# gillesdegottex/percivaltts

Hardware: AMD Instinct MI355X
Metric: acoustic frames/sec per WGAN-GP critic+gen step (higher is better)
Workload: dtype f32

## Files before the change

### include/percival_hip.h

```cpp
#ifndef PERCIVAL_HIP_H
#define PERCIVAL_HIP_H

#include <stddef.h>
#include <stdint.h>

#ifdef __cplusplus
extern "C" {
#endif

#define PTTS_OK            0
#define PTTS_EINVAL       -1
#define PTTS_ELAUNCH      -2
#define PTTS_EWORKSPACE   -3
#define PTTS_EDEVICE      -4

#define PTTS_IN_NONE     0
#define PTTS_IN_LRELU    1
#define PTTS_IN_MASKMUL  2

#define PTTS_PAD_SAME    0
#define PTTS_PAD_CAUSAL  1

#define PTTS_ACT_NONE    0
#define PTTS_ACT_LRELU   1
// ... 136 lines not shown
int ptts_dense_bf16x6_res(const float* A, const void* planes, const float* bias, float* C, int M, int N, int K,
                          long long lda, long long ldc, int in_mode, const float* in_scale, const float* in_shift,
                          const float* mask_src, float alpha, const float* res, int res_rows, long long ldr,
                          const float* out_mask, void* stream);
int ptts_dense_bf16x6_stats_rows(int M, int N);
int ptts_dense_bf16x6_stats(const float* A, const void* planes, const float* bias, float* C, int M, int N, int K,
                            long long lda, long long ldc, int in_mode, const float* in_scale, const float* in_shift,
                            float alpha, double* stats, int capacity_rows, int* nrows_out, void* stream);
int ptts_dense_bf16x6_bwd_affine(const float* A, const void* planes, float* C, int M, int N, int K, long long lda, long long ldc,
                                 const float* z, const float* scale, const float* shift, float alpha,
                                 double* stats, int capacity_rows, int* nrows_out, void* stream);
int ptts_partial_rows_sum(const double* partials, int nrows, int ncols, double* out, void* stream);
int ptts_dft_mirror(float* Ap, int NB, int B, int Cin, int Kh, void* stream);

int ptts_conv1d_freq_kernel_planes(const float* w, const float* tw, void* planes, int NB, int KW, int Cin, int N, int Kh, void* stream);

int ptts_transpose_batched(const float* src, float* dst, int nb, int rows, int cols, void* stream);
int ptts_conv1d_freq_wgrad_combine(const float* out2, float* dW, int KW, int Cin, int N, int Kh, void* stream);

size_t ptts_conv1d_freq_wgrad_inverse_workspace_bytes(int KW, int Cin, int N);
int ptts_conv1d_freq_wgrad_inverse(const float* Gt, const float* t2, float* dW, void* workspace, size_t workspace_bytes,
                                   int NB, int NBp, int KW, int Cin, int N, int Kh, void* stream);

int ptts_dense_bf16x6_batched(const float* A, long long strideA, const void* planes, long long stride_planes_bytes,
                              const float* bias, float* C, long long strideC, int nbatch, int M, int N, int K,
                              long long lda, long long ldc, int planes_count, void* stream);

int ptts_split3_frames(const float* x, void* p1, void* p2, void* p3, int B, int T, int C, int pad_left, int pad_right,
                       int Cp, void* stream);
int ptts_split3_weight_t(const float* w, void* p1, void* p2, void* p3, int KW, int C, int N, int Cp, void* stream);
int ptts_conv1d_bf16x6(const void* a1, const void* a2, const void* a3, const void* bt1, const void* bt2, const void* bt3,
                       const float* bias, float* y, int B, int T, int KW, int Cp, int N, void* stream);

int ptts_split3_frames_t(const float* x, void* p1, void* p2, void* p3, int B, int T, int C, int pad_left, int Tp, int Crows,
                         long long Pp, void* stream);
int ptts_conv1d_wgrad_bf16x6(const void* xt1, const void* xt2, const void* xt3, const void* yt1, const void* yt2,
                             const void* yt3, float* dw, int B, int T, int KW, int C, int N, int Crows, long long Pp,
                             void* stream);

int ptts_transpose_frames(const float* x, float* out, int B, int T, int C, int pad_left, int Tp, int Crows, long long Pp,
                          void* stream);
int ptts_conv1d_wgrad_t(const float* xt, const float* yt, float* dw, float* db, int B, int T, int KW, int C, int N, int Crows,
                        long long Pp, void* stream);

size_t ptts_colstats_workspace_bytes(long long rows, int C);
int ptts_colstats(const float* x, long long rows, int C,
// ... 144 lines not shown
```

### percivaltts_amd/_hip.py

```python
import ctypes
import os
import re

import torch

_HERE = os.path.dirname(os.path.abspath(__file__))
LIB_PATH = os.environ.get('PTTS_LIB_PATH') or os.path.join(_HERE, 'lib', 'libpercival_hip.so')
HEADER_PATH = os.environ.get('PTTS_HEADER_PATH') or os.path.join(_HERE, '..', 'include', 'percival_hip.h')


class HipLibraryError(RuntimeError):
    pass


_SCALARS = {'int': ctypes.c_int, 'unsigned': ctypes.c_uint, 'float': ctypes.c_float, 'double': ctypes.c_double,
            'size_t': ctypes.c_size_t, 'long long': ctypes.c_longlong, 'unsigned long long': ctypes.c_ulonglong}
_DECLARATOR = re.compile(r'(.*[\s*])(\w+)\s*(\[\s*\])?', re.S)


def _ctype(spelling, where):
    t = ' '.join(w for w in spelling.replace('*', ' * ').split() if w != 'const')
    if t.endswith('*'):
        return ctypes.c_char_p if t == 'char *' else ctypes.c_void_p
    if t not in _SCALARS:
# ... 32 lines not shown
        args = [] if m.group(3).strip() == 'void' else [_declaration(a, decl)[1] for a in m.group(3).split(',')]
        functions[m.group(2)] = (_ctype(m.group(1), decl), args)
    return structs, functions


def read_header(path):
    if not os.path.exists(path):
        raise HipLibraryError('percival_hip.h not found at {}: it lies in include/ beside the package (or set PTTS_HEADER_PATH). '
                              'The binding is read from it.'.format(path))
    with open(path) as f:
        return parse_header(f.read())


_STRUCTS, SIGNATURES = read_header(HEADER_PATH)


def _structure(name, cname):
    return type(name, (ctypes.Structure,), {'_fields_': _STRUCTS[cname], '__doc__': 'struct {} of include/percival_hip.h.'.format(cname)})


WGradDesc = _structure('WGradDesc', 'ptts_wgrad_desc')
DenseWgradReduceDesc = _structure('DenseWgradReduceDesc', 'ptts_dense_wgrad_reduce_desc')
DenseSplitDesc = _structure('DenseSplitDesc', 'ptts_dense_split_desc')
Conv2dReduceDesc = _structure('Conv2dReduceDesc', 'ptts_conv2d_reduce_desc')

_lib = None


def lib():
    global _lib
    if _lib is None:
        if not os.path.exists(LIB_PATH):
            raise HipLibraryError(
                'libpercival_hip.so not found at {}: run `python -c "import __graft_entry__ as g; g.build()"` '
                '(or `make -C percivaltts_amd/csrc`). There is no CPU fallback.'.format(LIB_PATH))
        l = ctypes.CDLL(LIB_PATH)
        for name, (res, args) in SIGNATURES.items():
            fn = getattr(l, name)
            fn.restype = res
            fn.argtypes = args
        if os.environ.get('PTTS_DETERMINISTIC', '0') == '1':
            l.ptts_set_deterministic(1)
        _lib = l
    return _lib


# ... 83 lines not shown
```

### percivaltts_amd/csrc/dense.hip

```cpp
#include "common.h"
#include <cstdlib>

namespace ptts {
namespace dns {

typedef __bf16 bf16x8 __attribute__((ext_vector_type(8)));
typedef __bf16 bf16x4 __attribute__((ext_vector_type(4)));
typedef __bf16 bf16x2 __attribute__((ext_vector_type(2)));
typedef float f32x4 __attribute__((ext_vector_type(4)));
typedef float f32x2 __attribute__((ext_vector_type(2)));
typedef unsigned u32x2 __attribute__((ext_vector_type(2)));
typedef unsigned short u16;

constexpr int THREADS = 512;
constexpr int NBLK = 256;
constexpr int BK = 32;

#define DNS_PRODUCTS(X) X(2, 0) X(1, 1) X(0, 2) X(1, 0) X(0, 1) X(0, 0)
#define DNS_PRODUCTS_NPL(NPL, X) do { if (NPL == 3) { X(2, 0) X(1, 1) X(0, 2) X(1, 0) X(0, 1) } X(0, 0) } while (0)

__device__ __forceinline__ unsigned pk_bf16(float a, float b) {
    return __builtin_bit_cast(unsigned, __builtin_convertvector((f32x2){a, b}, bf16x2));
}
__device__ __forceinline__ void split3_pair(float a, float b, unsigned& p1, unsigned& p2, unsigned& p3) {
    p1 = pk_bf16(a, b);
    const float ra = a - __builtin_bit_cast(float, p1 << 16), rb = b - __builtin_bit_cast(float, p1 & 0xffff0000u);
    p2 = pk_bf16(ra, rb);
    const float sa = ra - __builtin_bit_cast(float, p2 << 16), sb = rb - __builtin_bit_cast(float, p2 & 0xffff0000u);
    p3 = pk_bf16(sa, sb);
}
__device__ __forceinline__ float max_fast(float a, float b) {
    float r;
    asm("v_max_f32 %0, %1, %2" : "=v"(r) : "v"(a), "v"(b));
    return r;
// ... 171 lines not shown
#pragma unroll
        for (int h = 0; h < 4; ++h) split3_pair(v[2 * h], v[2 * h + 1], q[0][h], q[1][h], q[2][h]);
        const size_t idx = ((size_t)nt * a.KS + ks) * 64 + lane;
#pragma unroll
        for (int p = 0; p < 3; ++p)
            *reinterpret_cast<uint4*>(planes + p * ps + idx * 8) = make_uint4(q[p][0], q[p][1], q[p][2], q[p][3]);
    }
}

#ifndef DNS_DEPTH
#define DNS_DEPTH 2
#endif
struct DenseArgs {
    const float* A; const float* mask_src; const float* in_scale; const float* in_shift;
    const u16* planes; const float* bias; const float* out_mask; float* C;
    int M, N, K, NT, KS;
    long long lda, ldc;
    float alpha, out_alpha;
    int accumulate, has_affine, vec_out;
    const float* res; int res_rows; long long ldr;
    long long bsA, bsP, bsC;
    double* stats;
    const float* om_scale; const float* om_shift;
};

template <int MODE, bool AFFINE, int MT, int NPL>
__global__ __launch_bounds__(THREADS) void dense_bf16x6_kernel(DenseArgs g) {
    if (gridDim.z > 1) {
        g.A += (long long)blockIdx.z * g.bsA;
        g.planes += (long long)blockIdx.z * g.bsP;
        g.C += (long long)blockIdx.z * g.bsC;
    }
    constexpr int TBM = 16 * MT;
    constexpr int NA = (TBM * 8 + THREADS - 1) / THREADS;
    constexpr int ROWS = NA * THREADS / 8;
    constexpr int PL = ROWS * BK;
    constexpr bool MASK = MODE == PTTS_IN_MASKMUL;
    __shared__ __attribute__((aligned(16))) u16 As[2][NPL * PL];
    const int tid = threadIdx.x, lane = tid & 63;
    const int wave = __builtin_amdgcn_readfirstlane(tid >> 6);
    const int li = lane & 15, lg = lane >> 4;
    const int m0 = blockIdx.x * TBM, n0 = blockIdx.y * NBLK;
    const int KS = g.KS;
    const bool wave_live = n0 + 32 * wave < g.N;

    const int kq = tid & 7;
    const float* pa[NA]; const float* pm[NA]; bool oka[NA]; int dst[NA];
#pragma unroll
    for (int j = 0; j < NA; ++j) {
        const int row = (tid + j * THREADS) >> 3;
        oka[j] = row < TBM && m0 + row < g.M;
        const long long base = (long long)(oka[j] ? m0 + row : 0) * g.lda + 4 * kq;
        pa[j] = g.A + base;
        pm[j] = MASK ? g.mask_src + base : nullptr;
        dst[j] = row * BK + ((((kq >> 1) ^ ((row >> 1) & 2))) << 3) + (kq & 1) * 4;
// ... 35 lines not shown
                unsigned a1, a2, a3, b1, b2, b3;
                split3_pair(a[0], a[1], a1, a2, a3);
                split3_pair(a[2], a[3], b1, b2, b3);
                *reinterpret_cast<u32x2*>(d) = (u32x2){a1, b1};
                *reinterpret_cast<u32x2*>(d + PL) = (u32x2){a2, b2};
                *reinterpret_cast<u32x2*>(d + 2 * PL) = (u32x2){a3, b3};
            } else {
                *reinterpret_cast<u32x2*>(d) = (u32x2){pk_bf16(a[0], a[1]), pk_bf16(a[2], a[3])};
            }
        }
    };

    const size_t ps = (size_t)g.NT * KS * 512;
    const u16* wp[2];
#pragma unroll
    for (int j = 0; j < 2; ++j) wp[j] = g.planes + (((size_t)((n0 >> 4) + 2 * (wave_live ? wave : 0) + j) * KS) * 64 + lane) * 8;
    auto load_w = [&](int s, bf16x8 (&wf)[2][NPL]) {
#pragma unroll
        for (int j = 0; j < 2; ++j)
#pragma unroll
            for (int p = 0; p < NPL; ++p) wf[j][p] = *reinterpret_cast<const bf16x8*>(wp[j] + p * ps + (size_t)s * 512);
    };

    f32x4 acc[MT][2];
#pragma unroll
    for (int i = 0; i < MT; ++i) { acc[i][0] = f32x4{0.f, 0.f, 0.f, 0.f}; acc[i][1] = f32x4{0.f, 0.f, 0.f, 0.f}; }
    const int boff = li * BK + ((lg ^ ((li >> 1) & 2)) << 3);
    auto mfma_rows = [&](const u16* as, const bf16x8 (&wf)[2][NPL], int i0, int i1) {
#pragma unroll
        for (int i = i0; i < i1; ++i) {
            bf16x8 bf[NPL];
#pragma unroll
            for (int p = 0; p < NPL; ++p) bf[p] = *reinterpret_cast<const bf16x8*>(as + p * PL + boff + i * 16 * BK);
#define DNS_MM(PA, PW)                                                                                    \
            acc[i][0] = __builtin_amdgcn_mfma_f32_16x16x32_bf16(wf[0][PW < NPL ? PW : 0], bf[PA < NPL ? PA : 0], acc[i][0], 0, 0, 0);    \
            acc[i][1] = __builtin_amdgcn_mfma_f32_16x16x32_bf16(wf[1][PW < NPL ? PW : 0], bf[PA < NPL ? PA : 0], acc[i][1], 0, 0, 0);
            DNS_PRODUCTS_NPL(NPL, DNS_MM);
#undef DNS_MM
        }
    };

    constexpr int DEPTH = DNS_DEPTH;
    Stage sg[DEPTH];
    bf16x8 wc[2][NPL], wn[2][NPL];
#pragma unroll
    for (int j = 0; j < DEPTH; ++j) load_a(j, sg[j]);
    load_w(0, wc);
    commit(sg[0], As[0]);
    load_a(DEPTH, sg[0]);
    __syncthreads();
    auto step = [&](int s, int cut, Stage& nx) {
        const u16* as = As[s & 1];
        load_w(s + 1 < KS ? s + 1 : s, wn);
        mfma_rows(as, wc, 0, cut);
        commit(nx, As[(s + 1) & 1]);
        load_a(s + 1 + DEPTH, nx);
        mfma_rows(as, wc, cut, MT);
#pragma unroll
        for (int j = 0; j < 2; ++j)
#pragma unroll
            for (int p = 0; p < NPL; ++p) wc[j][p] = wn[j][p];
        __syncthreads();
    };
    auto run = [&](int cut) {
        int s = 0;
        for (; s + DEPTH <= KS; s += DEPTH) {
#pragma unroll
            for (int j = 0; j < DEPTH; ++j) step(s + j, cut, sg[(j + 1) % DEPTH]);
        }
#pragma unroll
        for (int j = 0; j < DEPTH; ++j)
            if (s + j < KS) step(s + j, cut, sg[(j + 1) % DEPTH]);
    };
    if (wave < 4) run(2); else run(MT - 2);
    if (!wave_live) return;
    const bool interior = m0 + TBM <= g.M;
    if (!g.vec_out) {
#pragma unroll
        for (int j = 0; j < 2; ++j)
#pragma unroll
            for (int i = 0; i < MT; ++i) {
                const int m = m0 + 16 * i + li;
                if (m >= g.M) continue;
#pragma unroll
                for (int e = 0; e < 4; ++e) {
                    const int n = n0 + 32 * wave + 16 * j + 4 * lg + e;
                    if (n >= g.N) continue;
                    const long long off = (long long)m * g.ldc + n;
                    float v = acc[i][j][e] + (g.bias ? g.bias[n] : 0.f);
                    if (g.out_mask) v *= g.out_mask[off] > 0.f ? 1.f : g.out_alpha;
                    if (g.res) { int mr = m; while (mr >= g.res_rows) mr -= g.res_rows; v += g.res[(long long)mr * g.ldr + n]; }
                    g.C[off] = v;
                }
            }
        return;
    }
#pragma unroll
    for (int j = 0; j < 2; ++j) {
        const int n = n0 + 32 * wave + 16 * j + 4 * lg;
        if (n >= g.N) continue;
        f32x4 bv = {0.f, 0.f, 0.f, 0.f};
        if (g.bias) bv = *reinterpret_cast<const f32x4*>(g.bias + n);
        const long long off0 = (long long)(m0 + li) * g.ldc + n;
        auto res_at = [&](int m) { int mr = m; while (mr >= g.res_rows) mr -= g.res_rows; return g.res + (long long)mr * g.ldr + n; };
        f32x4 ssum = {0.f, 0.f, 0.f, 0.f}, ssq = {0.f, 0.f, 0.f, 0.f};
        f32x4 osc = {1.f, 1.f, 1.f, 1.f}, osh = {0.f, 0.f, 0.f, 0.f};
        if (g.om_scale) { osc = *reinterpret_cast<const f32x4*>(g.om_scale + n); osh = *reinterpret_cast<const f32x4*>(g.om_shift + n); }
        auto aff_store = [&](f32x4& v, const f32x4& z) {
#pragma unroll
            for (int e = 0; e < 4; ++e) {
                const float gd = v[e] * ((z[e] * osc[e] + osh[e]) > 0.f ? 1.f : g.out_alpha);
                ssum[e] += gd * z[e]; ssq[e] += gd;
                v[e] = gd * osc[e];
            }
        };
        if (interior) {
            f32x4 mk[MT], old[MT];
            if (g.out_mask) {
#pragma unroll
                for (int i = 0; i < MT; ++i) mk[i] = *reinterpret_cast<const f32x4*>(g.out_mask + off0 + (long long)16 * i * g.ldc);
            }
            if (g.res) {
#pragma unroll
                for (int i = 0; i < MT; ++i) old[i] = *reinterpret_cast<const f32x4*>(res_at(m0 + 16 * i + li));
            }
#pragma unroll
            for (int i = 0; i < MT; ++i) {
                f32x4 v = acc[i][j] + bv;
                if (g.om_scale) {
                    aff_store(v, mk[i]);
                } else if (g.out_mask) {
#pragma unroll
                    for (int e = 0; e < 4; ++e) v[e] = v[e] * (mk[i][e] > 0.f ? 1.f : g.out_alpha);
                }
                if (g.res) v += old[i];
                if (g.stats && !g.om_scale) { ssum += v; ssq += v * v; }
                *reinterpret_cast<f32x4*>(g.C + off0 + (long long)16 * i * g.ldc) = v;
            }
        } else {
#pragma unroll
            for (int i = 0; i < MT; ++i) {
                const int m = m0 + 16 * i + li;
                if (m >= g.M) continue;
                const long long off = off0 + (long long)16 * i * g.ldc;
                f32x4 v = acc[i][j] + bv;
                if (g.out_mask) {
                    const f32x4 mk = *reinterpret_cast<const f32x4*>(g.out_mask + off);
                    if (g.om_scale) {
                        aff_store(v, mk);
                    } else {
#pragma unroll
                        for (int e = 0; e < 4; ++e) v[e] = v[e] * (mk[e] > 0.f ? 1.f : g.out_alpha);
                    }
                }
                if (g.res) v += *reinterpret_cast<const f32x4*>(res_at(m));
                if (g.stats && !g.om_scale) { ssum += v; ssq += v * v; }
                *reinterpret_cast<f32x4*>(g.C + off) = v;
            }
        }
        if (g.stats) {
#pragma unroll
            for (int e = 0; e < 4; ++e)
#pragma unroll
                for (int m = 1; m < 16; m <<= 1) { ssum[e] += __shfl_xor(ssum[e], m, 64); ssq[e] += __shfl_xor(ssq[e], m, 64); }
            if (li == 0) {
                double* row = g.stats + (size_t)blockIdx.x * 2 * g.N;
#pragma unroll
                for (int e = 0; e < 4; ++e) { row[n + e] = (double)ssum[e]; row[g.N + n + e] = (double)ssq[e]; }
            }
        }
    }
}

static int pick_mt(int M, int col_blocks) {
    static int forced = -1;
    if (forced < 0) { const char* e = getenv("PTTS_DENSE_MT"); forced = e ? atoi(e) : 0; }
    if (forced >= 4 && forced <= 8) return forced;
    int best = 8; double best_eff = -1.0;
    for (int mt = 4; mt <= 8; ++mt) {
        const long long blocks = (long long)((M + 16 * mt - 1) / (16 * mt)) * col_blocks;
// ... 370 lines not shown
                        const float* out_mask, double* stats, int stats_capacity_rows, int* stats_rows_out, void* stream) {
    const int accumulate = res != nullptr;
    PTTS_REQUIRE(!res || (res_rows > 0 && ldr >= N && M <= 8LL * res_rows), "dense_bf16x6: bad residual (rows %d, ldr %lld)", res_rows, ldr);
    PTTS_REQUIRE(A && planes && C, "dense_bf16x6: null matrix");
    PTTS_REQUIRE(ptts_dense_bf16x6_supported(M, N, K, lda, ldc), "dense_bf16x6: unsupported shape M=%d N=%d K=%d lda=%lld ldc=%lld (K and lda must be multiples of 4)", M, N, K, lda, ldc);
    PTTS_REQUIRE(lda >= K && ldc >= N, "dense_bf16x6: bad leading dims");
    PTTS_REQUIRE(in_mode >= 0 && in_mode <= 2, "dense_bf16x6: bad in_mode %d", in_mode);
    PTTS_REQUIRE((in_scale == nullptr) == (in_shift == nullptr), "dense_bf16x6: scale/shift must come together");
    PTTS_REQUIRE(in_mode != PTTS_IN_MASKMUL || mask_src, "dense_bf16x6: MASKMUL needs mask_src");
    PTTS_REQUIRE(in_mode == PTTS_IN_LRELU || !in_scale, "dense_bf16x6: scale/shift need PTTS_IN_LRELU");
    PTTS_REQUIRE(!(out_mask && bias), "dense_bf16x6: out_mask with bias is not defined");
    PTTS_REQUIRE(alpha >= 0.f && alpha <= 1.f, "dense_bf16x6: LeakyReLU slope %g outside [0, 1]", alpha);
    const bool vec_out = N % 4 == 0 && ldc % 4 == 0 && ((uintptr_t)C & 15) == 0 && (!bias || ((uintptr_t)bias & 15) == 0) &&
                         (!out_mask || ((uintptr_t)out_mask & 15) == 0) && (!res || (((uintptr_t)res & 15) == 0 && ldr % 4 == 0));
    PTTS_REQUIRE(((uintptr_t)A & 15) == 0 && (!mask_src || ((uintptr_t)mask_src & 15) == 0) &&
                 (!in_scale || (((uintptr_t)in_scale | (uintptr_t)in_shift) & 15) == 0), "dense_bf16x6: A, its mask and scale/shift must be 16-byte aligned");
    DenseArgs g;
    g.A = A; g.mask_src = mask_src; g.in_scale = in_scale; g.in_shift = in_shift; g.planes = (const u16*)planes; g.bias = bias;
    g.out_mask = out_mask; g.C = C; g.M = M; g.N = N; g.K = K;
    g.NT = (N + NBLK - 1) / NBLK * (NBLK / 16); g.KS = (K + BK - 1) / BK;
    g.lda = lda; g.ldc = ldc; g.alpha = alpha; g.out_alpha = alpha; g.accumulate = accumulate; g.has_affine = in_scale != nullptr; g.vec_out = vec_out;
    g.res = res; g.res_rows = res ? res_rows : 1; g.ldr = ldr;
    g.bsA = g.bsP = g.bsC = 0;
    const int cb = (N + NBLK - 1) / NBLK;
    const int mt = pick_mt(M, cb);
    const dim3 grid((unsigned)((M + 16 * mt - 1) / (16 * mt)), (unsigned)cb);
    g.stats = stats;
    g.om_scale = g_om_scale; g.om_shift = g_om_shift;
    if (stats) {
        PTTS_REQUIRE(vec_out, "dense_bf16x6_stats: N and ldc must be multiples of 4, C (and bias) 16-byte aligned");
        PTTS_REQUIRE(stats_capacity_rows >= (int)grid.x, "dense_bf16x6_stats: room for %d rows of sums, %d needed", stats_capacity_rows, (int)grid.x);
        *stats_rows_out = (int)grid.x;
    }
    hipStream_t st = (hipStream_t)stream;
    const bool one = ptts::bf16_products();
#define DNS_L(MODE, AFF, MT) do { if (one) hipLaunchKernelGGL((dense_bf16x6_kernel<MODE, AFF, MT, 1>), grid, dim3(THREADS), 0, st, g); \
                                  else hipLaunchKernelGGL((dense_bf16x6_kernel<MODE, AFF, MT, 3>), grid, dim3(THREADS), 0, st, g); } while (0)
#define DNS_M(MT)                                                                \
    do {                                                                         \
        if (in_mode == PTTS_IN_LRELU) { if (in_scale) DNS_L(PTTS_IN_LRELU, true, MT); else DNS_L(PTTS_IN_LRELU, false, MT); } \
        else if (in_mode == PTTS_IN_MASKMUL) DNS_L(PTTS_IN_MASKMUL, false, MT);  \
        else DNS_L(PTTS_IN_NONE, false, MT);                                     \
    } while (0)
    switch (mt) {
        case 4: DNS_M(4); break;
        case 5: DNS_M(5); break;
// ... 13 lines not shown
    const int NT = (N + NBLK - 1) / NBLK * (NBLK / 16), KS = (2 * Kh + BK - 1) / BK;
    const long long total = (long long)NT * KS * 64;
    const long long fstride = (long long)(ptts_dense_planes_bytes(N, 2 * Kh) / sizeof(u16));
    const dim3 grid((unsigned)((total + 255) / 256), (unsigned)((NB + WDFT_FCH - 1) / WDFT_FCH));
#define WDFT(KWv) hipLaunchKernelGGL(conv1d_wdft_planes_kernel<KWv>, grid, dim3(256), 0, (hipStream_t)stream, w, tw, (u16*)planes, fstride, NB, Cin, N, Kh, NT, KS)
    switch (KW) {
        case 3: WDFT(3); break;
        case 5: WDFT(5); break;
        case 7: WDFT(7); break;
        case 9: WDFT(9); break;
        case 11: WDFT(11); break;
        case 21: WDFT(21); break;
        default: set_error("conv1d_freq_kernel_planes: KW=%d not instantiated (3, 5, 7, 9, 11, 21)", KW); return PTTS_EINVAL;
    }
#undef WDFT
    return check_launch("conv1d_freq_kernel_planes");
}

extern "C" int ptts_dense_bf16x6_batched(const float* A, long long strideA, const void* planes, long long stride_planes_bytes,
                                         const float* bias, float* C, long long strideC, int nbatch, int M, int N, int K,
                                         long long lda, long long ldc, int planes_count, void* stream) {
    PTTS_REQUIRE(A && planes && C && nbatch > 0 && nbatch <= 65535, "dense_bf16x6_batched: bad arguments");
    PTTS_REQUIRE(ptts_dense_bf16x6_supported(M, N, K, lda, ldc), "dense_bf16x6_batched: unsupported shape M=%d N=%d K=%d lda=%lld ldc=%lld", M, N, K, lda, ldc);
    PTTS_REQUIRE(lda >= K && ldc >= N && planes_count >= 1 && planes_count <= 3 && planes_count != 2, "dense_bf16x6_batched: bad leading dims / planes");
    PTTS_REQUIRE(stride_planes_bytes % 16 == 0 && strideA % 4 == 0 && ((uintptr_t)A & 15) == 0, "dense_bf16x6_batched: strides of A / planes must keep 16-byte alignment");
    const bool vec_out = N % 4 == 0 && ldc % 4 == 0 && strideC % 4 == 0 && ((uintptr_t)C & 15) == 0 && (!bias || ((uintptr_t)bias & 15) == 0);
    DenseArgs g;
    g.A = A; g.mask_src = nullptr; g.in_scale = nullptr; g.in_shift = nullptr; g.planes = (const u16*)planes; g.bias = bias;
    g.out_mask = nullptr; g.C = C; g.M = M; g.N = N; g.K = K;
    g.NT = (N + NBLK - 1) / NBLK * (NBLK / 16); g.KS = (K + BK - 1) / BK;
    g.lda = lda; g.ldc = ldc; g.alpha = 0.f; g.out_alpha = 0.f; g.accumulate = 0; g.has_affine = 0; g.vec_out = vec_out;
    g.res = nullptr; g.res_rows = 1; g.ldr = 0;
    g.bsA = strideA; g.bsP = stride_planes_bytes / 2; g.bsC = strideC;
    g.stats = nullptr; g.om_scale = g.om_shift = nullptr;
    const int cb = (N + NBLK - 1) / NBLK;
    int mt = 8; double best_eff = -1.0;
    {
        static int forced = -1;
        if (forced < 0) { const char* e = getenv("PTTS_DENSE_BATCHED_MT"); forced = e ? atoi(e) : 0; }
        for (int m = 8; m >= 4; --m) {
            const int tiles = (M + 16 * m - 1) / (16 * m);
            const double eff = (double)M / (double)(tiles * 16 * m);
            if (eff > best_eff + 1e-9) { best_eff = eff; mt = m; }
        }
        if (forced >= 4 && forced <= 8) mt = forced;
    }
    const dim3 grid((unsigned)((M + 16 * mt - 1) / (16 * mt)), (unsigned)cb, (unsigned)nbatch);
    hipStream_t st = (hipStream_t)stream;
    const bool one = planes_count == 1;
#define DNS_B(MT) do { if (one) hipLaunchKernelGGL((dense_bf16x6_kernel<PTTS_IN_NONE, false, MT, 1>), grid, dim3(THREADS), 0, st, g); \
                       else hipLaunchKernelGGL((dense_bf16x6_kernel<PTTS_IN_NONE, false, MT, 3>), grid, dim3(THREADS), 0, st, g); } while (0)
    switch (mt) {
        case 4: DNS_B(4); break;
        case 5: DNS_B(5); break;
        case 6: DNS_B(6); break;
        case 7: DNS_B(7); break;
        default: DNS_B(8); break;
    }
#undef DNS_B
    return check_launch("dense_bf16x6_batched");
}

extern "C" int ptts_dense_wgrad_bf16x6_supported(int Kin, int N, int M, long long lda, long long ldb) {
    return (Kin > 0 && N > 0 && M > 0 && Kin % 4 == 0 && N % 4 == 0 && lda % 4 == 0 && ldb % 4 == 0 &&
            (long long)((Kin + WT - 1) / WT) * ((N + WT - 1) / WT) <= 65535) ? 1 : 0;
}

namespace {
int wgrad_split(int Kin, int N, int M) {
    const int tiles = ((Kin + WT - 1) / WT) * ((N + WT - 1) / WT), steps = (M + 31) / 32;
    int split = (256 + tiles - 1) / tiles;
    static int env_split = -1;
    if (env_split < 0) { const char* e = getenv("PTTS_DENSE_WGRAD_SPLIT"); env_split = e ? atoi(e) : 0; }
    if (env_split > 0) split = env_split;
    if (split > steps) split = steps;
    return split < 1 ? 1 : split;
}
}

extern "C" size_t ptts_dense_wgrad_workspace_bytes(int Kin, int N, int M) {
    if (Kin <= 0 || N <= 0 || M <= 0) return 0;
    const size_t tiles = (size_t)((Kin + WT - 1) / WT) * ((N + WT - 1) / WT);
// ... 83 lines not shown
```

### percivaltts_amd/ops.py

```python
import contextlib
import ctypes
import os

import torch

from . import _hip
from ._hip import call, ptr, stream, f32c, _workspace
from .ops_offline import *

IN_NONE, IN_LRELU, IN_MASKMUL = 0, 1, 2
PAD_SAME, PAD_CAUSAL = 0, 1
ACT_NONE, ACT_LRELU, ACT_SIGMOID, ACT_TANH = 0, 1, 2, 3
ACT_CODES = {None: ACT_NONE, 'linear': ACT_NONE, 'lrelu': ACT_LRELU, 'sigmoid': ACT_SIGMOID, 'tanh': ACT_TANH}


class Lazy(object):
    __slots__ = ('z', 'scale', 'shift', 'lrelu', 'alpha')

    def __init__(self, z, scale=None, shift=None, lrelu=False, alpha=0.3):
        self.z, self.scale, self.shift, self.lrelu, self.alpha = z, scale, shift, lrelu, alpha

    @property
    def shape(self):
        return self.z.shape

    def tensor(self):
        if self.scale is None and not self.lrelu:
            return self.z
        return affine_act(self.z, self.scale, self.shift, 'lrelu' if self.lrelu else None, self.alpha)


def as_lazy(v):
    return v if isinstance(v, Lazy) else Lazy(v)
# ... 1308 lines not shown

    @classmethod
    def clear(cls):
        cls.src = cls.key = cls.planes = None


def clear_caches():
    _C1Split.clear()
    _C1FFT.clear()
    _C1WgradT.clear()
    _C2M.clear()
    _C2C.clear()
    _DenseSplit.clear()
    _C1Cache.key = _C1Cache.ap = _C1Cache.y = None


class _C1FFT(object):
    default = os.environ.get('PTTS_CONV1D_FFT', '1') == '1'
    enabled = default
    KWS = (3, 5, 7, 9, 11, 21)
    wgrad_enabled = os.environ.get('PTTS_CONV1D_FFT_WGRAD', '1') == '1'
    bf16_one_product = os.environ.get('PTTS_CONV1D_FFT_BF16', '1') == '1'
    seg_target = int(os.environ.get('PTTS_CONV1D_FFT_SEG', '100'))
    consts = {}
    x_src = None; x_key = None; x_hat = None
    xw_src = None; xw_key = None; xw_planes = None
    w_hat = {}
    bufs = {}

    @staticmethod
    def eligible(a, w):
        B, T, Cin = a.shape
        KW, _, N = w.shape
        if not (a.is_cuda and B * T >= 4096 and KW >= 3 and KW % 2 == 1 and T % 4 == 0 and N % 4 == 0 and Cin >= 64):
            return False
        return B * (T // _C1FFT.segment(T, KW)) <= 65535

    @classmethod
    def segment(cls, T, KW):
        tgt = cls.seg_target
        if tgt <= 0:
            return T
        best = T
        for S in range(4, T + 1, 4):
            if T % S == 0 and S >= 2 * KW and abs(S - tgt) < abs(best - tgt):
                best = S
# ... 47 lines not shown
        T2 = torch.zeros(2 * KW, NBp, dtype=torch.float64)
        T2[:KW, :NB] = (torch.cos(tk) * cf.view(NB, 1) / P).t()
        T2[KW:, :NB] = (torch.sin(tk) * cf.view(NB, 1) / P).t()
        TP = (2 * KW + 15) // 16 * 16
        T2f = torch.zeros(NB, TP, dtype=torch.float64)
        T2f[:, :2 * KW] = T2[:, :NB].t()
        to = lambda m: m.to(torch.float32).to(dev).contiguous()
        c = {'S': S, 'NS': NS, 'P': P, 'NB': NB, 'R': R, 'Rp': Rp, 'NBp': NBp, 'TP': TP, 'pl': pl, 'Kh': (Cin + 7) // 8 * 8,
             'D': to(D), 'E': to(E), 'Tw': to(Tw), 'T2': to(T2), 'T2f': to(T2f)}
        cls.consts[key] = c
        return c

    @classmethod
    def x_transform(cls, a, KW):
        B, T, Cin = a.shape
        key = (a._version, tuple(a.shape), KW, _hip.stream_id())
        if cls.x_src is a and cls.x_key == key:
            return cls.x_hat
        c = cls.const(T, KW, Cin, a.device)
        NB, Kh, NS, S, P = c['NB'], c['Kh'], c['NS'], c['S'], c['P']
        Z = B * NS
        Ap = cls._buf('Ap', (B, T, Cin, KW, S), NB * 2 * Z * 2 * Kh, a.device)
        lib = _hip.lib()
        npb = lib.ptts_dense_planes_bytes(Cin, P)
        xpl = cls._scratch('xpl', Z * npb, a.device)
        call('ptts_split3_frame_windows', ptr(a), B, T, Cin, NS, S, -c['pl'], P, P, ptr(xpl), npb, stream(), tag=('x', Z))
        call('ptts_dense_bf16x6_batched', ptr(c['D']), 0, ptr(xpl), npb, None, ptr(Ap), 2 * Kh, Z, c['R'], Cin, P, P, Z * 2 * Kh, 3, stream(),
             tag=('dft', Z, c['R'], Cin, P))
        call('ptts_dft_mirror', ptr(Ap), NB, Z, Cin, Kh, stream())
        cls.x_src, cls.x_key, cls.x_hat = a, key, Ap
        return Ap

    @classmethod
    def kernel(cls, w, T):
        KW, Cin, N = w.shape
        flat = getattr(w, '_ptts_flat', None)
        epoch = None if flat is None else flat.epoch
        sid = _hip.stream_id()
        c = cls.const(T, KW, Cin, w.device)
        NB, Kh = c['NB'], c['Kh']
        geo = (c['S'], NB, Kh)
        ent = cls.w_hat.get((id(w), sid))
        if ent is not None and ent[0] is w and ent[1] == w._version and ent[2] == epoch and flat is not None and ent[5] == geo:
            if cls.frozen_log is not None and id(flat) in cls.frozen:
                cls.frozen_log.append((w, ent[4], T))
            return ent[4]
        lib = _hip.lib()
        npb = lib.ptts_dense_planes_bytes(N, 2 * Kh)
        if ent is not None and ent[0] is w and ent[5] == geo:
            planes = ent[4]
        else:
            planes = torch.empty(NB * npb, dtype=torch.uint8, device=w.device)
# ... 19 lines not shown
    frozen_log = None

    @classmethod
    def refresh_planes(cls, items):
        for w, planes, T in items:
            KW, Cin, N = w.shape
            cls._build_kernel_planes(w, cls.const(T, KW, Cin, w.device), planes)
        return len(items)

    @classmethod
    def forward(cls, a, w, b, y):
        B, T, Cin = a.shape
        KW, _, N = w.shape
        c = cls.const(T, KW, Cin, a.device)
        NB, Kh, NS, S = c['NB'], c['Kh'], c['NS'], c['S']
        Z = B * NS
        lib = _hip.lib()
        Ap = cls.x_transform(a, KW)
        wpl = cls.kernel(w, T)
        npw = lib.ptts_dense_planes_bytes(N, 2 * Kh)
        Yh = cls._scratch('Yh', NB * 2 * Z * N * 4, a.device)
        call('ptts_dense_bf16x6_batched', ptr(Ap), 2 * Z * 2 * Kh, ptr(wpl), npw, None, ptr(Yh), 2 * Z * N, NB, 2 * Z, N, 2 * Kh,
             2 * Kh, N, 1 if _Flags.bf16_products else 3, stream(), tag=('freq', NB, 2 * Z, N, 2 * Kh))
        npy = lib.ptts_dense_planes_bytes(N, c['R'])
        ypl = cls._scratch('ypl', Z * npy, a.device)
        call('ptts_split3_dense_weight_strided', ptr(Yh), N, ptr(ypl), npy, Z, Z * N, c['R'], N, 0, stream(), tag=('y', Z))
        call('ptts_dense_bf16x6_batched', ptr(c['E']), 0, ptr(ypl), npy, ptr(b), ptr(y), S * N, Z, S, N, c['Rp'], c['Rp'], N, 3, stream(),
             tag=('idft', Z, S, N, c['Rp']))

    @classmethod
    def has_x(cls, a, KW):
        return a is not None and cls.x_src is a and cls.x_key == (a._version, tuple(a.shape), KW, _hip.stream_id())

    @classmethod
    def wgrad(cls, a, dy, KW):
        B, T, Cin = a.shape
        N = dy.shape[-1]
        c = cls.const(T, KW, Cin, a.device)
        NB, Kh, NS, S, P = c['NB'], c['Kh'], c['NS'], c['S'], c['P']
        Z = B * NS
        lib = _hip.lib()
        dev = a.device
        Ap = cls.x_hat
        npx = lib.ptts_dense_planes_bytes(2 * Kh, 2 * Z)
        if cls.xw_src is not a or cls.xw_key != cls.x_key or cls.xw_planes is None:
            xw = cls._scratch('xw', NB * npx, dev)
            call('ptts_split3_dense_weight_strided', ptr(Ap), 2 * Z * 2 * Kh, ptr(xw), npx, NB, 2 * Kh, 2 * Z, 2 * Kh, 0, stream(), tag=('xw', NB))
            cls.xw_src, cls.xw_key, cls.xw_planes = a, cls.x_key, xw
        npd = lib.ptts_dense_planes_bytes(N, P)
        dpl = cls._scratch('dpl', Z * npd, dev)
        call('ptts_split3_frame_windows', ptr(dy), B, T, N, NS, S, 0, P, S, ptr(dpl), npd, stream(), tag=('dy', Z))
        DYh = cls._scratch('DYh', NB * 2 * Z * N * 4, dev)
        call('ptts_dense_bf16x6_batched', ptr(c['D']), 0, ptr(dpl), npd, None, ptr(DYh), N, Z, c['R'], N, P, P, Z * N, 3, stream(),
             tag=('dft_dy', Z, c['R'], N, P))
        DYt = cls._scratch('DYt', NB * N * 2 * Z * 4, dev)
        call('ptts_transpose_batched', ptr(DYh), ptr(DYt), NB, 2 * Z, N, stream())
        Gt = cls._scratch('Gt', NB * N * 2 * Kh * 4, dev)
        call('ptts_dense_bf16x6_batched', ptr(DYt), N * 2 * Z, ptr(cls.xw_planes), npx, None, ptr(Gt), N * 2 * Kh, NB, N, 2 * Kh, 2 * Z,
             2 * Z, 2 * Kh, 1 if _Flags.bf16_products else 3, stream(), tag=('corr', NB, N, 2 * Kh, 2 * Z))
        dw = torch.empty((KW, Cin, N), dtype=torch.float32, device=dev)
        if KW in cls.KWS:
            ws = _workspace(lib.ptts_conv1d_freq_wgrad_inverse_workspace_bytes(KW, Cin, N), dev)
            call('ptts_conv1d_freq_wgrad_inverse', ptr(Gt), ptr(c['T2f']), ptr(dw), ptr(ws), ws.numel(), NB, c['TP'], KW, Cin, N, Kh, stream(),
                 tag=(NB, KW, Cin, N))
        else:
            out2 = torch.empty(2 * KW * N * 2 * Kh, dtype=torch.float32, device=dev)
            gemm_raw(c['T2'], Gt[:NB * N * 2 * Kh * 4].view(torch.float32), out2, 2 * KW, N * 2 * Kh, NB, lda=c['NBp'], ldb=N * 2 * Kh, ldc=N * 2 * Kh)
            call('ptts_conv1d_freq_wgrad_combine', ptr(out2), ptr(dw), KW, Cin, N, Kh, stream())
        return dw

    @classmethod
    def clear(cls):
        cls.x_src = cls.x_key = cls.x_hat = None
        cls.xw_src = cls.xw_key = cls.xw_planes = None
        cls.w_hat = {k: (e if id(getattr(e[0], '_ptts_flat', None)) in cls.frozen else (e[0], None, None, e[3], e[4], e[5]) + tuple(e[6:]))
                     for k, e in cls.w_hat.items()}

# ... 716 lines not shown
```

Measured before the change: 4.717 million.

## Fuse bf16x3 splitting of the B operand and the DFT mirror into the dense kernel

```diff
diff --git a/include/percival_hip.h b/include/percival_hip.h
--- a/include/percival_hip.h
+++ b/include/percival_hip.h
@@ -182,6 +182,13 @@
 int ptts_conv1d_freq_wgrad_inverse(const float* Gt, const float* t2, float* dW, void* workspace, size_t workspace_bytes,
                                    int NB, int NBp, int KW, int Cin, int N, int Kh, void* stream);
 
+#define PTTS_DENSE_ROWS 0
+typedef struct ptts_dense_rows_desc {
+    const float* src;
+    long long ld, stride;
+    int windows, T, NS, S, row_off, kvalid;
+    int mirror_kh, reserved;
+} ptts_dense_rows_desc;
 int ptts_dense_bf16x6_batched(const float* A, long long strideA, const void* planes, long long stride_planes_bytes,
                               const float* bias, float* C, long long strideC, int nbatch, int M, int N, int K,
                               long long lda, long long ldc, int planes_count, void* stream);
diff --git a/percivaltts_amd/_hip.py b/percivaltts_amd/_hip.py
--- a/percivaltts_amd/_hip.py
+++ b/percivaltts_amd/_hip.py
@@ -78,6 +78,7 @@
 WGradDesc = _structure('WGradDesc', 'ptts_wgrad_desc')
 DenseWgradReduceDesc = _structure('DenseWgradReduceDesc', 'ptts_dense_wgrad_reduce_desc')
 DenseSplitDesc = _structure('DenseSplitDesc', 'ptts_dense_split_desc')
+DenseRowsDesc = _structure('DenseRowsDesc', 'ptts_dense_rows_desc')
 Conv2dReduceDesc = _structure('Conv2dReduceDesc', 'ptts_conv2d_reduce_desc')
 
 _lib = None
diff --git a/percivaltts_amd/csrc/dense.hip b/percivaltts_amd/csrc/dense.hip
--- a/percivaltts_amd/csrc/dense.hip
+++ b/percivaltts_amd/csrc/dense.hip
@@ -10,6 +10,7 @@
 typedef float f32x4 __attribute__((ext_vector_type(4)));
 typedef float f32x2 __attribute__((ext_vector_type(2)));
 typedef unsigned u32x2 __attribute__((ext_vector_type(2)));
+typedef unsigned u32x4 __attribute__((ext_vector_type(4)));
 typedef unsigned short u16;
 
 constexpr int THREADS = 512;
@@ -227,15 +228,23 @@
     long long bsA, bsP, bsC;
     double* stats;
     const float* om_scale; const float* om_shift;
+    const float* Brows; long long ldb, bsB;
+    int bwin, bT, bNS, bS, brow_off, bkvalid;
+    int bvec;
+    int mirror_kh;
 };
-
-template <int MODE, bool AFFINE, int MT, int NPL>
+constexpr int BROW = NBLK + 2;
+constexpr int BTILE = BK * BROW;
+constexpr size_t BROWS_LDS_BYTES = 2 * BTILE * sizeof(float);
+
+template <int MODE, bool AFFINE, int MT, int NPL, int BSRC = 0>
 __global__ __launch_bounds__(THREADS) void dense_bf16x6_kernel(DenseArgs g) {
     if (gridDim.z > 1) {
         g.A += (long long)blockIdx.z * g.bsA;
         g.planes += (long long)blockIdx.z * g.bsP;
         g.C += (long long)blockIdx.z * g.bsC;
     }
+    extern __shared__ __attribute__((aligned(16))) float Bt[];
     constexpr int TBM = 16 * MT;
     constexpr int NA = (TBM * 8 + THREADS - 1) / THREADS;
     constexpr int ROWS = NA * THREADS / 8;
@@ -317,6 +326,69 @@
             for (int p = 0; p < NPL; ++p) wf[j][p] = *reinterpret_cast<const bf16x8*>(wp[j] + p * ps + (size_t)s * 512);
     };
 
+    long long brow0 = 0; int bk_lo = 0, bk_hi = 0;
+    if (BSRC) {
+        if (g.bwin) {
+            const int z = blockIdx.z, b = z / g.bNS, r0 = g.brow_off + (z - b * g.bNS) * g.bS;
+            brow0 = ((long long)b * g.bT + r0) * g.ldb;
+            bk_lo = r0 < 0 ? -r0 : 0;
+            bk_hi = min(min(g.bkvalid, g.bT - r0), g.K);
+        } else {
+            brow0 = (long long)blockIdx.z * g.bsB;
+            bk_hi = g.bkvalid > 0 ? min(g.bkvalid, g.K) : g.K;
+        }
+    }
+    f32x4 vb[BSRC ? 4 : 1];
+    auto load_b = [&](int s) {
+#pragma unroll
+        for (int j = 0; j < 4; ++j) {
+            const int k = s * BK + wave + 8 * j;
+            const bool kok = k >= bk_lo && k < bk_hi;
+            const float* row = g.Brows + (kok ? brow0 + (long long)k * g.ldb : 0LL);
+            f32x4 v;
+            if (g.bvec) {
+                const int n = n0 + 4 * lane;
+                const bool ok = kok && n < g.N;
+                v = *reinterpret_cast<const f32x4*>(row + (n < g.N ? n : 0));
+                if (!ok) v = f32x4{0.f, 0.f, 0.f, 0.f};
+            } else {
+#pragma unroll
+                for (int c = 0; c < 4; ++c) {
+                    const int n = n0 + lane + 64 * c;
+                    const float x = row[n < g.N ? n : 0];
+                    v[c] = (kok && n < g.N) ? x : 0.f;
+                }
+            }
+            vb[j] = v;
+        }
+    };
+    auto store_b = [&](float* bt) {
+#pragma unroll
+        for (int j = 0; j < 4; ++j) {
+            float* d = bt + (wave + 8 * j) * BROW;
+            if (g.bvec) {
+                *reinterpret_cast<f32x2*>(d + 4 * lane) = f32x2{vb[j][0], vb[j][1]};
+                *reinterpret_cast<f32x2*>(d + 4 * lane + 2) = f32x2{vb[j][2], vb[j][3]};
+            } else {
+#pragma unroll
+                for (int c = 0; c < 4; ++c) d[lane + 64 * c] = vb[j][c];
+            }
+        }
+    };
+    auto frag_b = [&](const float* bt, bf16x8 (&wf)[2][NPL]) {
+#pragma unroll
+        for (int j = 0; j < 2; ++j) {
+            float v[8];
+#pragma unroll
+            for (int e = 0; e < 8; ++e) v[e] = bt[(8 * lg + e) * BROW + 32 * wave + 16 * j + li];
+            unsigned q[3][4];
+#pragma unroll
+            for (int h = 0; h < 4; ++h) split3_pair(v[2 * h], v[2 * h + 1], q[0][h], q[1][h], q[2][h]);
+#pragma unroll
+            for (int p = 0; p < NPL; ++p) wf[j][p] = __builtin_bit_cast(bf16x8, (u32x4){q[p][0], q[p][1], q[p][2], q[p][3]});
+        }
+    };
+
     f32x4 acc[MT][2];
 #pragma unroll
     for (int i = 0; i < MT; ++i) { acc[i][0] = f32x4{0.f, 0.f, 0.f, 0.f}; acc[i][1] = f32x4{0.f, 0.f, 0.f, 0.f}; }
@@ -340,24 +412,36 @@
     bf16x8 wc[2][NPL], wn[2][NPL];
 #pragma unroll
     for (int j = 0; j < DEPTH; ++j) load_a(j, sg[j]);
-    load_w(0, wc);
+    if (BSRC) load_b(0); else load_w(0, wc);
     commit(sg[0], As[0]);
     load_a(DEPTH, sg[0]);
+    if (BSRC) { store_b(Bt); load_b(1); }
     __syncthreads();
-    auto step = [&](int s, int cut, Stage& nx) {
+    if (BSRC) {
+        frag_b(Bt, wc);
+        store_b(Bt + BTILE);
+        load_b(2);
+        __syncthreads();
+    }
+    auto step = [&](int s, int cut, Stage& nx) __attribute__((always_inline)) {
         const u16* as = As[s & 1];
-        load_w(s + 1 < KS ? s + 1 : s, wn);
+        if (!BSRC) load_w(s + 1 < KS ? s + 1 : s, wn);
         mfma_rows(as, wc, 0, cut);
         commit(nx, As[(s + 1) & 1]);
         load_a(s + 1 + DEPTH, nx);
+        if (BSRC) { store_b(Bt + (s & 1) * BTILE); load_b(s + 3); }
         mfma_rows(as, wc, cut, MT);
-#pragma unroll
-        for (int j = 0; j < 2; ++j)
-#pragma unroll
-            for (int p = 0; p < NPL; ++p) wc[j][p] = wn[j][p];
+        if (BSRC) {
+            frag_b(Bt + ((s + 1) & 1) * BTILE, wc);
+        } else {
+#pragma unroll
+            for (int j = 0; j < 2; ++j)
+#pragma unroll
+                for (int p = 0; p < NPL; ++p) wc[j][p] = wn[j][p];
+        }
         __syncthreads();
     };
-    auto run = [&](int cut) {
+    auto run = [&](int cut) __attribute__((always_inline)) {
         int s = 0;
         for (; s + DEPTH <= KS; s += DEPTH) {
 #pragma unroll
@@ -386,6 +470,7 @@
                     if (g.out_mask) v *= g.out_mask[off] > 0.f ? 1.f : g.out_alpha;
                     if (g.res) { int mr = m; while (mr >= g.res_rows) mr -= g.res_rows; v += g.res[(long long)mr * g.ldr + n]; }
                     g.C[off] = v;
+                    if (BSRC && g.mirror_kh) g.C[(long long)(m ^ 1) * g.ldc + g.mirror_kh + n] = (m & 1) ? -v : v;
                 }
             }
         return;
@@ -394,6 +479,21 @@
     for (int j = 0; j < 2; ++j) {
         const int n = n0 + 32 * wave + 16 * j + 4 * lg;
         if (n >= g.N) continue;
+        if (BSRC && n + 4 > g.N) {
+#pragma unroll
+            for (int i = 0; i < MT; ++i) {
+                const int m = m0 + 16 * i + li;
+                if (m >= g.M) continue;
+#pragma unroll
+                for (int e = 0; e < 4; ++e) {
+                    if (n + e >= g.N) continue;
+                    const float v = acc[i][j][e] + (g.bias ? g.bias[n + e] : 0.f);
+                    g.C[(long long)m * g.ldc + n + e] = v;
+                    if (g.mirror_kh) g.C[(long long)(m ^ 1) * g.ldc + g.mirror_kh + n + e] = (m & 1) ? -v : v;
+                }
+            }
+            continue;
+        }
         f32x4 bv = {0.f, 0.f, 0.f, 0.f};
         if (g.bias) bv = *reinterpret_cast<const f32x4*>(g.bias + n);
         const long long off0 = (long long)(m0 + li) * g.ldc + n;
@@ -409,6 +509,9 @@
                 v[e] = gd * osc[e];
             }
         };
+        auto mirror_store = [&](int m, const f32x4& v) {
+            *reinterpret_cast<f32x4*>(g.C + (long long)(m ^ 1) * g.ldc + g.mirror_kh + n) = (m & 1) ? -v : v;
+        };
         if (interior) {
             f32x4 mk[MT], old[MT];
             if (g.out_mask) {
@@ -431,6 +534,7 @@
                 if (g.res) v += old[i];
                 if (g.stats && !g.om_scale) { ssum += v; ssq += v * v; }
                 *reinterpret_cast<f32x4*>(g.C + off0 + (long long)16 * i * g.ldc) = v;
+                if (BSRC && g.mirror_kh) mirror_store(m0 + 16 * i + li, v);
             }
         } else {
 #pragma unroll
@@ -451,6 +555,7 @@
                 if (g.res) v += *reinterpret_cast<const f32x4*>(res_at(m));
                 if (g.stats && !g.om_scale) { ssum += v; ssq += v * v; }
                 *reinterpret_cast<f32x4*>(g.C + off) = v;
+                if (BSRC && g.mirror_kh) mirror_store(m, v);
             }
         }
         if (g.stats) {
@@ -867,6 +972,7 @@
     g.lda = lda; g.ldc = ldc; g.alpha = alpha; g.out_alpha = alpha; g.accumulate = accumulate; g.has_affine = in_scale != nullptr; g.vec_out = vec_out;
     g.res = res; g.res_rows = res ? res_rows : 1; g.ldr = ldr;
     g.bsA = g.bsP = g.bsC = 0;
+    g.Brows = nullptr; g.ldb = g.bsB = 0; g.bwin = g.bT = g.bNS = g.bS = g.brow_off = g.bkvalid = g.bvec = g.mirror_kh = 0;
     const int cb = (N + NBLK - 1) / NBLK;
     const int mt = pick_mt(M, cb);
     const dim3 grid((unsigned)((M + 16 * mt - 1) / (16 * mt)), (unsigned)cb);
@@ -926,10 +1032,32 @@
                                          long long lda, long long ldc, int planes_count, void* stream) {
     PTTS_REQUIRE(A && planes && C && nbatch > 0 && nbatch <= 65535, "dense_bf16x6_batched: bad arguments");
     PTTS_REQUIRE(ptts_dense_bf16x6_supported(M, N, K, lda, ldc), "dense_bf16x6_batched: unsupported shape M=%d N=%d K=%d lda=%lld ldc=%lld", M, N, K, lda, ldc);
-    PTTS_REQUIRE(lda >= K && ldc >= N && planes_count >= 1 && planes_count <= 3 && planes_count != 2, "dense_bf16x6_batched: bad leading dims / planes");
+    PTTS_REQUIRE(lda >= K && ldc >= N && planes_count >= 0 && planes_count <= 3 && planes_count != 2, "dense_bf16x6_batched: bad leading dims / planes");
     PTTS_REQUIRE(stride_planes_bytes % 16 == 0 && strideA % 4 == 0 && ((uintptr_t)A & 15) == 0, "dense_bf16x6_batched: strides of A / planes must keep 16-byte alignment");
-    const bool vec_out = N % 4 == 0 && ldc % 4 == 0 && strideC % 4 == 0 && ((uintptr_t)C & 15) == 0 && (!bias || ((uintptr_t)bias & 15) == 0);
+    const bool vec_out = (N % 4 == 0 || planes_count == PTTS_DENSE_ROWS) && ldc % 4 == 0 && strideC % 4 == 0 && ((uintptr_t)C & 15) == 0 &&
+                         (!bias || ((uintptr_t)bias & 15) == 0);
     DenseArgs g;
+    g.Brows = nullptr; g.ldb = g.bsB = 0; g.bwin = g.bT = g.bNS = g.bS = g.brow_off = g.bkvalid = g.bvec = g.mirror_kh = 0;
+    const bool rows = planes_count == PTTS_DENSE_ROWS;
+    if (rows) {
+        const ptts_dense_rows_desc& d = *static_cast<const ptts_dense_rows_desc*>(planes);
+        PTTS_REQUIRE(d.src && d.ld >= N, "dense_bf16x6_batched: rows operand without a source, or ld=%lld < N=%d", d.ld, N);
+        if (d.windows) {
+            PTTS_REQUIRE(d.T > 0 && d.NS > 0 && d.S > 0 && d.kvalid > 0 && nbatch % d.NS == 0, "dense_bf16x6_batched: bad windows (T=%d NS=%d S=%d kvalid=%d for %d products)", d.T, d.NS, d.S, d.kvalid, nbatch);
+        } else {
+            PTTS_REQUIRE(d.stride >= 0 && d.kvalid >= 0, "dense_bf16x6_batched: negative stride or row count of the rows operand");
+        }
+        if (d.mirror_kh) {
+            PTTS_REQUIRE(d.mirror_kh > 0 && d.mirror_kh % 4 == 0 && d.mirror_kh >= N && ldc >= d.mirror_kh + N && M % 2 == 0 && !bias,
+                         "dense_bf16x6_batched: mirror store needs Kh %% 4 == 0, N <= Kh, Kh + N <= ldc, an even M and no bias (Kh=%d N=%d M=%d ldc=%lld)", d.mirror_kh, N, M, ldc);
+            PTTS_REQUIRE(nbatch == 1 || strideC >= d.mirror_kh + N || strideC >= (long long)M * ldc, "dense_bf16x6_batched: the mirror columns would overlap the next product's");
+        }
+        g.Brows = d.src; g.ldb = d.ld; g.bsB = d.stride;
+        g.bwin = d.windows ? 1 : 0; g.bT = d.T; g.bNS = d.NS; g.bS = d.S; g.brow_off = d.row_off; g.bkvalid = d.kvalid;
+        g.bvec = (N % 4 == 0 && d.ld % 4 == 0 && (d.windows || d.stride % 4 == 0) && ((uintptr_t)d.src & 15) == 0) ? 1 : 0;
+        g.mirror_kh = d.mirror_kh;
+        planes = nullptr;
+    }
     g.A = A; g.mask_src = nullptr; g.in_scale = nullptr; g.in_shift = nullptr; g.planes = (const u16*)planes; g.bias = bias;
     g.out_mask = nullptr; g.C = C; g.M = M; g.N = N; g.K = K;
     g.NT = (N + NBLK - 1) / NBLK * (NBLK / 16); g.KS = (K + BK - 1) / BK;
@@ -952,7 +1080,12 @@
     const dim3 grid((unsigned)((M + 16 * mt - 1) / (16 * mt)), (unsigned)cb, (unsigned)nbatch);
     hipStream_t st = (hipStream_t)stream;
     const bool one = planes_count == 1;
-#define DNS_B(MT) do { if (one) hipLaunchKernelGGL((dense_bf16x6_kernel<PTTS_IN_NONE, false, MT, 1>), grid, dim3(THREADS), 0, st, g); \
+#define DNS_R(MT) do { static bool attr = false;                                                                                    \
+        if (!attr) { (void)hipFuncSetAttribute(reinterpret_cast<const void*>(&dense_bf16x6_kernel<PTTS_IN_NONE, false, MT, 3, 1>),  \
+                                               hipFuncAttributeMaxDynamicSharedMemorySize, (int)BROWS_LDS_BYTES); attr = true; }    \
+        hipLaunchKernelGGL((dense_bf16x6_kernel<PTTS_IN_NONE, false, MT, 3, 1>), grid, dim3(THREADS), BROWS_LDS_BYTES, st, g); } while (0)
+#define DNS_B(MT) do { if (rows) DNS_R(MT);                                                                                         \
+                       else if (one) hipLaunchKernelGGL((dense_bf16x6_kernel<PTTS_IN_NONE, false, MT, 1>), grid, dim3(THREADS), 0, st, g); \
                        else hipLaunchKernelGGL((dense_bf16x6_kernel<PTTS_IN_NONE, false, MT, 3>), grid, dim3(THREADS), 0, st, g); } while (0)
     switch (mt) {
         case 4: DNS_B(4); break;
@@ -962,6 +1095,7 @@
         default: DNS_B(8); break;
     }
 #undef DNS_B
+#undef DNS_R
     return check_launch("dense_bf16x6_batched");
 }
 
diff --git a/percivaltts_amd/ops.py b/percivaltts_amd/ops.py
--- a/percivaltts_amd/ops.py
+++ b/percivaltts_amd/ops.py
@@ -9,6 +9,20 @@
 from .ops_offline import *
 
 IN_NONE, IN_LRELU, IN_MASKMUL = 0, 1, 2
+DENSE_ROWS = 0
+
+
+def _rows_desc(src, ld, stride=0, kvalid=0, windows=None, mirror_kh=0):
+    d = _hip.DenseRowsDesc()
+    d.src, d.ld, d.stride, d.kvalid, d.mirror_kh = src.data_ptr(), ld, stride, kvalid, mirror_kh
+    if windows is not None:
+        d.windows = 1
+        d.T, d.NS, d.S, d.row_off, d.kvalid = windows
+    return d
+
+
+def _desc_ptr(d):
+    return ctypes.cast(ctypes.pointer(d), ctypes.c_void_p)
 PAD_SAME, PAD_CAUSAL = 0, 1
 ACT_NONE, ACT_LRELU, ACT_SIGMOID, ACT_TANH = 0, 1, 2, 3
 ACT_CODES = {None: ACT_NONE, 'linear': ACT_NONE, 'lrelu': ACT_LRELU, 'sigmoid': ACT_SIGMOID, 'tanh': ACT_TANH}
@@ -1363,6 +1377,8 @@
     wgrad_enabled = os.environ.get('PTTS_CONV1D_FFT_WGRAD', '1') == '1'
     bf16_one_product = os.environ.get('PTTS_CONV1D_FFT_BF16', '1') == '1'
     seg_target = int(os.environ.get('PTTS_CONV1D_FFT_SEG', '100'))
+    fused = os.environ.get('PTTS_CONV1D_FFT_FUSED', '1') == '1'
+    fused_dy = os.environ.get('PTTS_CONV1D_FFT_FUSED_DY', '0') == '1'
     consts = {}
     x_src = None; x_key = None; x_hat = None
     xw_src = None; xw_key = None; xw_planes = None
@@ -1456,12 +1472,17 @@
         Z = B * NS
         Ap = cls._buf('Ap', (B, T, Cin, KW, S), NB * 2 * Z * 2 * Kh, a.device)
         lib = _hip.lib()
-        npb = lib.ptts_dense_planes_bytes(Cin, P)
-        xpl = cls._scratch('xpl', Z * npb, a.device)
-        call('ptts_split3_frame_windows', ptr(a), B, T, Cin, NS, S, -c['pl'], P, P, ptr(xpl), npb, stream(), tag=('x', Z))
-        call('ptts_dense_bf16x6_batched', ptr(c['D']), 0, ptr(xpl), npb, None, ptr(Ap), 2 * Kh, Z, c['R'], Cin, P, P, Z * 2 * Kh, 3, stream(),
-             tag=('dft', Z, c['R'], Cin, P))
-        call('ptts_dft_mirror', ptr(Ap), NB, Z, Cin, Kh, stream())
+        if cls.fused:
+            d = _rows_desc(a, Cin, windows=(T, NS, S, -c['pl'], P), mirror_kh=Kh)
+            call('ptts_dense_bf16x6_batched', ptr(c['D']), 0, _desc_ptr(d), 0, None, ptr(Ap), 2 * Kh, Z, c['R'], Cin, P, P, Z * 2 * Kh,
+                 DENSE_ROWS, stream(), tag=('dft', Z, c['R'], Cin, P))
+        else:
+            npb = lib.ptts_dense_planes_bytes(Cin, P)
+            xpl = cls._scratch('xpl', Z * npb, a.device)
+            call('ptts_split3_frame_windows', ptr(a), B, T, Cin, NS, S, -c['pl'], P, P, ptr(xpl), npb, stream(), tag=('x', Z))
+            call('ptts_dense_bf16x6_batched', ptr(c['D']), 0, ptr(xpl), npb, None, ptr(Ap), 2 * Kh, Z, c['R'], Cin, P, P, Z * 2 * Kh, 3, stream(),
+                 tag=('dft', Z, c['R'], Cin, P))
+            call('ptts_dft_mirror', ptr(Ap), NB, Z, Cin, Kh, stream())
         cls.x_src, cls.x_key, cls.x_hat = a, key, Ap
         return Ap
 
@@ -1527,6 +1548,11 @@
         Yh = cls._scratch('Yh', NB * 2 * Z * N * 4, a.device)
         call('ptts_dense_bf16x6_batched', ptr(Ap), 2 * Z * 2 * Kh, ptr(wpl), npw, None, ptr(Yh), 2 * Z * N, NB, 2 * Z, N, 2 * Kh,
              2 * Kh, N, 1 if _Flags.bf16_products else 3, stream(), tag=('freq', NB, 2 * Z, N, 2 * Kh))
+        if cls.fused:
+            d = _rows_desc(Yh, Z * N, stride=N, kvalid=c['R'])
+            call('ptts_dense_bf16x6_batched', ptr(c['E']), 0, _desc_ptr(d), 0, ptr(b), ptr(y), S * N, Z, S, N, c['Rp'], c['Rp'], N,
+                 DENSE_ROWS, stream(), tag=('idft', Z, S, N, c['Rp']))
+            return
         npy = lib.ptts_dense_planes_bytes(N, c['R'])
         ypl = cls._scratch('ypl', Z * npy, a.device)
         call('ptts_split3_dense_weight_strided', ptr(Yh), N, ptr(ypl), npy, Z, Z * N, c['R'], N, 0, stream(), tag=('y', Z))
@@ -1552,12 +1578,17 @@
             xw = cls._scratch('xw', NB * npx, dev)
             call('ptts_split3_dense_weight_strided', ptr(Ap), 2 * Z * 2 * Kh, ptr(xw), npx, NB, 2 * Kh, 2 * Z, 2 * Kh, 0, stream(), tag=('xw', NB))
             cls.xw_src, cls.xw_key, cls.xw_planes = a, cls.x_key, xw
-        npd = lib.ptts_dense_planes_bytes(N, P)
-        dpl = cls._scratch('dpl', Z * npd, dev)
-        call('ptts_split3_frame_windows', ptr(dy), B, T, N, NS, S, 0, P, S, ptr(dpl), npd, stream(), tag=('dy', Z))
         DYh = cls._scratch('DYh', NB * 2 * Z * N * 4, dev)
-        call('ptts_dense_bf16x6_batched', ptr(c['D']), 0, ptr(dpl), npd, None, ptr(DYh), N, Z, c['R'], N, P, P, Z * N, 3, stream(),
-             tag=('dft_dy', Z, c['R'], N, P))
+        if cls.fused and cls.fused_dy:
+            d = _rows_desc(dy, N, windows=(T, NS, S, 0, S))
+            call('ptts_dense_bf16x6_batched', ptr(c['D']), 0, _desc_ptr(d), 0, None, ptr(DYh), N, Z, c['R'], N, P, P, Z * N, DENSE_ROWS, stream(),
+                 tag=('dft_dy', Z, c['R'], N, P))
+        else:
+            npd = lib.ptts_dense_planes_bytes(N, P)
+            dpl = cls._scratch('dpl', Z * npd, dev)
+            call('ptts_split3_frame_windows', ptr(dy), B, T, N, NS, S, 0, P, S, ptr(dpl), npd, stream(), tag=('dy', Z))
+            call('ptts_dense_bf16x6_batched', ptr(c['D']), 0, ptr(dpl), npd, None, ptr(DYh), N, Z, c['R'], N, P, P, Z * N, 3, stream(),
+                 tag=('dft_dy', Z, c['R'], N, P))
         DYt = cls._scratch('DYt', NB * N * 2 * Z * 4, dev)
         call('ptts_transpose_batched', ptr(DYh), ptr(DYt), NB, 2 * Z, N, stream())
         Gt = cls._scratch('Gt', NB * N * 2 * Kh * 4, dev)
```

Result: no change. 4.758 million, median of 6 (+0.9%).
